# thilinarmtb/lsbench

Measured on AMD Instinct MI355X. Metric: cg_solves_per_sec, higher is better.
Workload: dtype f64

## Files before the change

lsbench_amd/csrc/hip_kernels.hip:

```cpp
#include "hip_kcommon.h"

__device__ __forceinline__ void spmv_publish(double *__restrict__ partials, double dot,
                                             double *sred, const lsb_ar_tail &tail) {
  if (!partials)
    return;
  double d[1] = {dot};
  wg_sum<1>(d, sred);
  if (tail.counter)
    ar_tail(partials, d[0], tail);
  else if (threadIdx.x == 0)
    partials[blockIdx.x] = d[0];
}

enum { SP_PREFETCH = 1, SP_NT = 2 };

template <int FLAGS, class T>
__device__ __forceinline__ T stream_load(const T *p) {
  if (FLAGS & SP_NT)
    return __builtin_nontemporal_load(p);
  return *p;
}

#define LSB_ISSUE_BLOCK(kk)                                                    \
  do {                                                                         \
    r0 = rowblk[kk], r1 = rowblk[(kk) + 1];                                    \
    j0 = offs[r0], j1 = offs[r1];                                              \
    if (j1 - j0 <= CAP) {                                                      \
      _Pragma("unroll") for (int u = 0; u < U; u++) {                          \
        const int t = (int)tid + u * WG;                                       \
        if (t < j1 - j0) {                                                     \
          c[u] = stream_load<FLAGS>(cols + j0 + t);                            \
          v[u] = stream_load<FLAGS>(vals + j0 + t);                            \
        }                                                                      \
      }                                                                        \
    }                                                                          \
  } while (0)

template <int CAP, int FLAGS, class VT = double>
__global__ __launch_bounds__(WG, 8) void k_spmv_adaptive(
    const int *__restrict__ rowblk, const unsigned char *__restrict__ blklanes,
    unsigned nblk, const int *__restrict__ offs, const int *__restrict__ cols,
    const VT *__restrict__ vals, const double *__restrict__ x,
    double *__restrict__ y, const double *__restrict__ xdot,
    double *__restrict__ partials, const lsb_pcg_state *__restrict__ st,
    const int *__restrict__ rowmap, const lsb_ar_tail tail) {
  __shared__ double sprod[CAP];
  __shared__ double sred[4];
  const unsigned tid = threadIdx.x;
  const unsigned gx = gridDim.x / NXCD;
  const unsigned xcd = blockIdx.x % NXCD, slot = blockIdx.x / NXCD;
  const unsigned chunk = (nblk + NXCD - 1) / NXCD;
  const unsigned kbeg = xcd * chunk, kend = min(kbeg + chunk, nblk);
  constexpr int U = CAP / WG;
  double dot = 0.0;
  int c[U];
  VT v[U];
  int r0 = 0, r1 = 0, j0 = 0, j1 = 0;
  unsigned k = kbeg + slot;
  if (k < kend)
    LSB_ISSUE_BLOCK(k);
  if (st && st->status)
    return;
  for (; k < kend; k += gx) {
    const int cr0 = r0, cj0 = j0, cnt = j1 - j0, nr = r1 - r0;
    if (cnt <= CAP) {
#pragma unroll
      for (int u = 0; u < U; u++) {
        const int t = (int)tid + u * WG;
        if (t < cnt)
          sprod[t] = (double)v[u] * x[c[u]];
      }
      if ((FLAGS & SP_PREFETCH) && k + gx < kend)
        LSB_ISSUE_BLOCK(k + gx);
      __syncthreads();
      unsigned L;
      if (blklanes) {
        L = blklanes[k];
      } else {
        L = 1;
        while (L < 64 && (unsigned)nr * (L * 2) <= WG)
          L <<= 1;
      }
      const unsigned sl = tid / L, l = tid % L, slots = WG / L;
      for (unsigned rb = 0; rb < (unsigned)nr; rb += slots) {
        const unsigned r = rb + sl;
        double s = 0.0;
        if (r < (unsigned)nr) {
          const int a = offs[cr0 + r] - cj0, b = offs[cr0 + r + 1] - cj0;
          for (int j = a + (int)l; j < b; j += (int)L)
            s += sprod[j];
        }
        for (unsigned off = L >> 1; off > 0; off >>= 1)
          s += __shfl_xor(s, off, 64);
        if (r < (unsigned)nr && l == 0) {
          if (rowmap) {
            y[rowmap[cr0 + r]] += s;
          } else {
            y[cr0 + r] = s;
            if (xdot)
              dot += s * xdot[cr0 + r];
          }
        }
      }
      __syncthreads();
    } else {
      double s[1] = {0.0};
      for (int j = cj0 + (int)tid; j < cj0 + cnt; j += WG)
        s[0] += (double)vals[j] * x[cols[j]];
      wg_sum<1>(s, sred);
      if (tid == 0) {
        if (rowmap) {
          y[rowmap[cr0]] += s[0];
        } else {
          y[cr0] = s[0];
          if (xdot)
            dot += s[0] * xdot[cr0];
        }
      }
      if ((FLAGS & SP_PREFETCH) && k + gx < kend)
        LSB_ISSUE_BLOCK(k + gx);
    }
    if (!(FLAGS & SP_PREFETCH) && k + gx < kend)
      LSB_ISSUE_BLOCK(k + gx);
  }
  spmv_publish(partials, dot, sred, tail);
}
#undef LSB_ISSUE_BLOCK

template <int L, class VT = double>
__global__ __launch_bounds__(WG) void k_spmv_subwave(
    unsigned n, unsigned rows_per_wg, const int *__restrict__ offs,
    const int *__restrict__ cols, const VT *__restrict__ vals,
    const double *__restrict__ x, double *__restrict__ y,
    const double *__restrict__ xdot, double *__restrict__ partials,
    const lsb_pcg_state *__restrict__ st) {
  __shared__ double sred[4];
  const unsigned tid = threadIdx.x, slot = tid / L, l = tid % L;
  constexpr unsigned SLOTS = WG / L;
  const unsigned w = xcd_contiguous_wg();
  const unsigned ra = min(w * rows_per_wg, n), rb = min(ra + rows_per_wg, n);
  const int stopped = st ? st->status : 0;
  double dot = 0.0;
  for (unsigned base = ra; base < rb; base += SLOTS) {
    const unsigned r = base + slot;
    double s = 0.0, xd = 0.0;
    if (r < rb) {
      const int j0 = offs[r], j1 = offs[r + 1];
      if (xdot)
        xd = xdot[r];
      for (int j = j0 + (int)l; j < j1; j += L)
        s += (double)vals[j] * x[cols[j]];
    }
#pragma unroll
    for (int off = L >> 1; off > 0; off >>= 1)
      s += __shfl_xor(s, off, 64);
    if (stopped)
      return;
    if (r < rb && l == 0) {
      y[r] = s;
      dot += s * xd;
    }
  }
  if (stopped)
    return;
  if (partials) {
    double d[1] = {dot};
    wg_sum<1>(d, sred);
    if (tid == 0)
      partials[w] = d[0];
  }
}

template <int L>
__global__ __launch_bounds__(WG) void k_spmv_subwave_p(
    unsigned n, unsigned rows_per_wg, const int *__restrict__ offs,
    const int *__restrict__ cols, const double *__restrict__ vals,
    const double *__restrict__ r, const double *__restrict__ dinv, double dc,
    const double *__restrict__ pold, double *__restrict__ pnew, double *__restrict__ y,
    double *__restrict__ partials, lsb_pcg_state *__restrict__ st, int parity,
    const double *__restrict__ parts2, unsigned nparts2) {
  __shared__ double sred[8];
  const unsigned tid = threadIdx.x, slot = tid / L, l = tid % L;
  constexpr unsigned SLOTS = WG / L;
  const unsigned w = xcd_contiguous_wg();
  const unsigned ra = min(w * rows_per_wg, n), rb = min(ra + rows_per_wg, n);
  const int stopped = st->status;
  const double rz_old = st->rz[parity], thresh2 = st->thresh2;
  double v[2];
  wg_sum_partials<2>(parts2, nparts2, v, sred);
  if (stopped)
    return;
  const double rz_new = v[0], rr = v[1];
  const bool conv = rr <= thresh2;
  if (blockIdx.x == 0 && threadIdx.x == 0) {
    const int it = st->iters + 1;
    st->iters = it;
    st->rr = rr;
    st->rz[parity ^ 1] = rz_new;
    if (conv)
      st->status = LSB_STATUS_CONVERGED;
    else if (it >= st->maxit)
      st->status = LSB_STATUS_MAXIT;
  }
  if (conv)
    return;
  const double beta = rz_new / rz_old;
  double dot = 0.0;
  for (unsigned base = ra; base < rb; base += SLOTS) {
    const unsigned row = base + slot;
    double s = 0.0, pi = 0.0;
    if (row < rb) {
      const int j0 = offs[row], j1 = offs[row + 1];
      pi = pnew_of(dinv ? dinv[row] : dc, r[row], beta, pold[row]);
      for (int j = j0 + (int)l; j < j1; j += L) {
        const int c = cols[j];
        s += vals[j] * pnew_of(dinv ? dinv[c] : dc, r[c], beta, pold[c]);
      }
    }
#pragma unroll
    for (int off = L >> 1; off > 0; off >>= 1)
      s += __shfl_xor(s, off, 64);
    if (row < rb && l == 0) {
      pnew[row] = pi;
      y[row] = s;
      dot += s * pi;
    }
  }
  double d[1] = {dot};
  wg_sum<1>(d, sred);
  if (tid == 0)
    partials[w] = d[0];
}

__global__ __launch_bounds__(WG) void k_spmv_scalar(
    unsigned n, unsigned rows_per_wg, const int *__restrict__ offs,
    const int *__restrict__ cols, const double *__restrict__ vals,
    const double *__restrict__ x, double *__restrict__ y,
    const double *__restrict__ xdot, double *__restrict__ partials,
    const lsb_pcg_state *__restrict__ st) {
  if (st && st->status)
    return;
  __shared__ double sred[4];
  const unsigned w = xcd_contiguous_wg();
  const unsigned ra = min(w * rows_per_wg, n), rb = min(ra + rows_per_wg, n);
  double dot = 0.0;
  for (unsigned r = ra + threadIdx.x; r < rb; r += WG) {
    double s = 0.0;
    for (int j = offs[r]; j < offs[r + 1]; j++)
      s += vals[j] * x[cols[j]];
    y[r] = s;
    if (xdot)
      dot += s * xdot[r];
  }
  if (partials) {
    double d[1] = {dot};
    wg_sum<1>(d, sred);
    if (threadIdx.x == 0)
      partials[w] = d[0];
  }
}

struct sell_deal {
  unsigned turns, base, L, period, full, total, colturns;
};
__device__ __forceinline__ sell_deal sell_deal_init(unsigned ns, unsigned period, unsigned xcd) {
  sell_deal d;
  d.period = period, d.full = 0, d.total = 0, d.colturns = 0;
  if (!period) {
    const unsigned ngrp = (ns + 3) / 4, chunk = (ngrp + NXCD - 1) / NXCD;
    const unsigned g0 = min(xcd * chunk, ngrp), g1 = min(g0 + chunk, ngrp);
    d.base = g0 * 4, d.turns = g1 - g0, d.L = 0;
  } else {
    const unsigned qlo = period * xcd / NXCD, qhi = period * (xcd + 1) / NXCD;
    const unsigned planes = ns / period, rem = ns % period;
    d.L = qhi - qlo, d.base = qlo;
    d.full = d.L * planes;
    d.total = d.full + (rem > qlo ? min(qhi, rem) - qlo : 0u);
    d.colturns = (planes / 4) * d.L;
    d.turns = d.colturns + (d.total - 4 * d.colturns + 3) / 4;
  }
  return d;
}
__device__ __forceinline__ unsigned sell_deal_slice(const sell_deal &d, unsigned it, unsigned wave,
                                                    unsigned ns) {
  if (!d.period) {
    const unsigned si = d.base + it * 4 + wave;
    return si < ns ? si : 0xFFFFFFFFu;
  }
  if (it < d.colturns)
    return ((it / d.L) * 4 + wave) * d.period + d.base + it % d.L;
  const unsigned m = it * 4 + wave;
  if (m >= d.total)
    return 0xFFFFFFFFu;
  if (m < d.full)
    return (m / d.L) * d.period + d.base + m % d.L;
  return (ns / d.period) * d.period + d.base + (m - d.full);
}

typedef int i2v __attribute__((ext_vector_type(2)));
typedef int i4v __attribute__((ext_vector_type(4)));
typedef double sell_d2u __attribute__((ext_vector_type(2), aligned(8)));
typedef double sell_d2v __attribute__((ext_vector_type(2)));
#define SELL_U 5
template <class VT> struct vt2;
template <> struct vt2<double> { typedef double type __attribute__((ext_vector_type(2))); };
template <> struct vt2<float> { typedef float type __attribute__((ext_vector_type(2))); };
template <int FLAGS, class VT = double>
__global__ __launch_bounds__(WG, 6) void k_spmv_sell(
    const unsigned *__restrict__ sptr, unsigned s0, unsigned ns, unsigned period, unsigned n,
    const int *__restrict__ cols, const VT *__restrict__ vals,
    const double *__restrict__ x, double *__restrict__ y, const double *__restrict__ xdot,
    double *__restrict__ partials, const lsb_pcg_state *__restrict__ st, const lsb_ar_tail tail) {
  __shared__ double sred[4];
  const unsigned tid = threadIdx.x, lane = tid & 63u, wave = tid >> 6;
  const unsigned gx = gridDim.x / NXCD, xcd = blockIdx.x % NXCD, slot = blockIdx.x / NXCD;
  const sell_deal deal = sell_deal_init(ns, period, xcd);
  const int stopped = st ? st->status : 0;
  double dot = 0.0;
  for (unsigned g = slot; g < deal.turns; g += gx) {
    const unsigned si = __builtin_amdgcn_readfirstlane(sell_deal_slice(deal, g, wave, ns));
    if (si != 0xFFFFFFFFu) {
      const unsigned s = s0 + si;
      const unsigned base = sptr[s], len = (sptr[s + 1] - base) / LSB_SELL_ROWS;
      typedef typename vt2<VT>::type v2t;
      const i2v *cp = (const i2v *)(cols + base) + lane;
      const v2t *vp = (const v2t *)(vals + base) + lane;
      double a0 = 0.0, a1 = 0.0;
      for (unsigned j0 = 0; j0 < len; j0 += SELL_U) {
        i2v c[SELL_U];
        v2t v[SELL_U];
#pragma unroll
        for (int u = 0; u < SELL_U; u++)
          if (j0 + u < len) {
            if (FLAGS & SP_NT) {
              c[u] = __builtin_nontemporal_load(cp + (size_t)(j0 + u) * 64);
              v[u] = __builtin_nontemporal_load(vp + (size_t)(j0 + u) * 64);
            } else {
              c[u] = cp[(size_t)(j0 + u) * 64];
              v[u] = vp[(size_t)(j0 + u) * 64];
            }
          }
        if (stopped)
          return;
#pragma unroll
        for (int u = 0; u < SELL_U; u++)
          if (j0 + u < len) {
            a0 = fma((double)v[u].x, x[c[u].x], a0);
            a1 = fma((double)v[u].y, x[c[u].y], a1);
          }
      }
      const unsigned row = s * LSB_SELL_ROWS + 2 * lane;
      if (row + 1 < n) {
        const sell_d2v o = {a0, a1};
        *(sell_d2v *)(y + row) = o;
        if (xdot) {
          dot = fma(a0, xdot[row], dot);
          dot = fma(a1, xdot[row + 1], dot);
        }
      } else if (row < n) {
        y[row] = a0;
        if (xdot)
          dot = fma(a0, xdot[row], dot);
      }
    }
  }
  if (stopped)
    return;
  spmv_publish(partials, dot, sred, tail);
}

typedef short s2v __attribute__((ext_vector_type(2)));
template <int FLAGS, class VT = double, bool CHEB = false>
__global__ __launch_bounds__(WG, 6) void k_spmv_sell16(
    const unsigned *__restrict__ sptr, unsigned s0, unsigned ns, unsigned period, unsigned n,
    unsigned row_begin, unsigned xlen, const short *__restrict__ codes, const int *__restrict__ sbase,
    const VT *__restrict__ vals, const double *__restrict__ vconst, unsigned ulen,
    const double *__restrict__ x, double *__restrict__ y, const double *__restrict__ xdot,
    double *__restrict__ partials,
    const lsb_pcg_state *__restrict__ st, const lsb_ar_tail tail, const lsb_cheb_epi epi) {
  __shared__ double sred[4];
  const unsigned tid = threadIdx.x, lane = tid & 63u, wave = tid >> 6;
  const unsigned gx = gridDim.x / NXCD, xcd = blockIdx.x % NXCD, slot = blockIdx.x / NXCD;
  const sell_deal deal = sell_deal_init(ns, period, xcd);
  const int stopped = st ? st->status : 0;
  double dot = 0.0;
  for (unsigned g = slot; g < deal.turns; g += gx) {
    const unsigned si = __builtin_amdgcn_readfirstlane(sell_deal_slice(deal, g, wave, ns));
    if (si != 0xFFFFFFFFu) {
      const unsigned s = s0 + si;
      typedef typename vt2<VT>::type v2t;
      const unsigned base = ulen ? s * ulen * LSB_SELL_ROWS : sptr[s];
      const unsigned len = ulen ? ulen : (sptr[s + 1] - base) / LSB_SELL_ROWS;
      const unsigned q0 = base / LSB_SELL_ROWS;
      const unsigned row = s * LSB_SELL_ROWS + 2 * lane;
      const int grow = (int)(row + row_begin);
      double a0 = 0.0, a1 = 0.0;
      sell_d2v xd = {0.0, 0.0};
      if (!CHEB && xdot) {
        if (row + 1 < n)
          xd = *(const sell_d2v *)(xdot + row);
        else if (row < n)
          xd.x = xdot[row];
      }
      for (unsigned j0 = 0; j0 < len; j0 += SELL_U) {
        if (vconst) {
          const unsigned cnt = len - j0 < SELL_U ? len - j0 : SELL_U;
          i4v rec[SELL_U];
          double cst[SELL_U];
#pragma unroll
          for (int u = 0; u < SELL_U; u++) {
            const unsigned q = q0 + j0 + ((unsigned)u < cnt ? (unsigned)u : cnt - 1u);
            rec[u] = ((const i4v *)sbase)[q];
            cst[u] = vconst[q];
          }
          bool fast = true;
#pragma unroll
          for (int u = 0; u < SELL_U; u++)
            fast = fast && (rec[u].y < 0 && rec[u].z < 0);
          if (fast) {
            if (stopped)
              return;
            sell_d2u t[SELL_U];
#pragma unroll
            for (int u = 0; u < SELL_U; u++)
              t[u] = *(const sell_d2u *)(x + (grow + rec[u].x));
#pragma unroll
            for (int u = 0; u < SELL_U; u++)
              if ((unsigned)u < cnt) {
                const VT cv = (VT)cst[u];
// ... 1332 lines not shown
```

Measured before the change: 1.159.

## Prefetch row offsets and lane counts for next block in adaptive SpMV

Splits the block-issue macro into metadata and stream parts, and computes the lane log2 for the next block ahead of time (reading blklanes via readfirstlane). It also prefetches each thread's row offsets for the first two reduction passes into registers, which takes the dependent offs loads off the critical path after the barrier. x gathers are batched in groups of four so more loads are in flight at once. In exchange it uses more registers, which may lower occupancy, and the group loop assumes U is a multiple of GB.

```diff
diff --git a/lsbench_amd/csrc/hip_kernels.hip b/lsbench_amd/csrc/hip_kernels.hip
--- a/lsbench_amd/csrc/hip_kernels.hip
+++ b/lsbench_amd/csrc/hip_kernels.hip
@@ -21,10 +21,20 @@
   return *p;
 }
 
-#define LSB_ISSUE_BLOCK(kk)                                                    \
+#define LSB_ISSUE_META(kk)                                                     \
   do {                                                                         \
     r0 = rowblk[kk], r1 = rowblk[(kk) + 1];                                    \
     j0 = offs[r0], j1 = offs[r1];                                              \
+    if (blklanes) {                                                            \
+      lg = (unsigned)__ffs(__builtin_amdgcn_readfirstlane((int)blklanes[kk])) - 1u;  \
+    } else {                                                                   \
+      lg = 0;                                                                  \
+      while (lg < 6 && ((unsigned)(r1 - r0) << (lg + 1)) <= WG)                \
+        lg++;                                                                  \
+    }                                                                          \
+  } while (0)
+#define LSB_ISSUE_STREAM()                                                     \
+  do {                                                                         \
     if (j1 - j0 <= CAP) {                                                      \
       _Pragma("unroll") for (int u = 0; u < U; u++) {                          \
         const int t = (int)tid + u * WG;                                       \
@@ -33,6 +43,23 @@
           v[u] = stream_load<FLAGS>(vals + j0 + t);                            \
         }                                                                      \
       }                                                                        \
+    }                                                                          \
+  } while (0)
+
+#define LSB_ISSUE_BLOCK(kk)                                                    \
+  do {                                                                         \
+    LSB_ISSUE_META(kk);                                                        \
+    LSB_ISSUE_STREAM();                                                        \
+  } while (0)
+
+#define LSB_ISSUE_OFFS()                                                       \
+  do {                                                                         \
+    if (j1 - j0 <= CAP) {                                                      \
+      const unsigned rows = (unsigned)(r1 - r0), sn = tid >> lg, step = WG >> lg; \
+      if (sn < rows)                                                           \
+        ro[0] = offs[r0 + sn], ro[1] = offs[r0 + sn + 1];                      \
+      if (sn + step < rows)                                                    \
+        ro[2] = offs[r0 + sn + step], ro[3] = offs[r0 + sn + step + 1];        \
     }                                                                          \
   } while (0)
 
@@ -52,41 +79,51 @@
   const unsigned chunk = (nblk + NXCD - 1) / NXCD;
   const unsigned kbeg = xcd * chunk, kend = min(kbeg + chunk, nblk);
   constexpr int U = CAP / WG;
+  constexpr int GB = 4;
   double dot = 0.0;
-  int c[U];
+  int c[U] = {};
   VT v[U];
+  int ro[4] = {0, 0, 0, 0};
   int r0 = 0, r1 = 0, j0 = 0, j1 = 0;
+  unsigned lg = 0;
   unsigned k = kbeg + slot;
-  if (k < kend)
+  if (k < kend) {
     LSB_ISSUE_BLOCK(k);
+    LSB_ISSUE_OFFS();
+  }
   if (st && st->status)
     return;
   for (; k < kend; k += gx) {
     const int cr0 = r0, cj0 = j0, cnt = j1 - j0, nr = r1 - r0;
+    const unsigned clg = lg;
     if (cnt <= CAP) {
 #pragma unroll
-      for (int u = 0; u < U; u++) {
-        const int t = (int)tid + u * WG;
-        if (t < cnt)
-          sprod[t] = (double)v[u] * x[c[u]];
+      for (int h = 0; cnt > 0 && h < U; h += GB) {
+        double xv[GB];
+#pragma unroll
+        for (int u = 0; u < GB; u++)
+          xv[u] = x[c[h + u]];
+#pragma unroll
+        for (int u = 0; u < GB; u++) {
+          const int t = (int)tid + (h + u) * WG;
+          if (t < cnt)
+            sprod[t] = (double)v[h + u] * xv[u];
+        }
       }
       if ((FLAGS & SP_PREFETCH) && k + gx < kend)
         LSB_ISSUE_BLOCK(k + gx);
       __syncthreads();
-      unsigned L;
-      if (blklanes) {
-        L = blklanes[k];
-      } else {
-        L = 1;
-        while (L < 64 && (unsigned)nr * (L * 2) <= WG)
-          L <<= 1;
-      }
-      const unsigned sl = tid / L, l = tid % L, slots = WG / L;
-      for (unsigned rb = 0; rb < (unsigned)nr; rb += slots) {
+      const unsigned L = 1u << clg, sl = tid >> clg, l = tid & (L - 1u), slots = WG >> clg;
+      unsigned pass = 0;
+      for (unsigned rb = 0; rb < (unsigned)nr; rb += slots, pass++) {
         const unsigned r = rb + sl;
         double s = 0.0;
         if (r < (unsigned)nr) {
-          const int a = offs[cr0 + r] - cj0, b = offs[cr0 + r + 1] - cj0;
+          int a, b;
+          if (pass < 2)
+            a = (pass ? ro[2] : ro[0]) - cj0, b = (pass ? ro[3] : ro[1]) - cj0;
+          else
+            a = offs[cr0 + r] - cj0, b = offs[cr0 + r + 1] - cj0;
           for (int j = a + (int)l; j < b; j += (int)L)
             s += sprod[j];
         }
@@ -121,10 +158,17 @@
         LSB_ISSUE_BLOCK(k + gx);
     }
     if (!(FLAGS & SP_PREFETCH) && k + gx < kend)
-      LSB_ISSUE_BLOCK(k + gx);
+      LSB_ISSUE_META(k + gx);
+    if (k + gx < kend)
+      LSB_ISSUE_OFFS();
+    if (!(FLAGS & SP_PREFETCH) && k + gx < kend)
+      LSB_ISSUE_STREAM();
   }
   spmv_publish(partials, dot, sred, tail);
 }
+#undef LSB_ISSUE_OFFS
+#undef LSB_ISSUE_META
+#undef LSB_ISSUE_STREAM
 #undef LSB_ISSUE_BLOCK
 
 template <int L, class VT = double>
```

Measured after the change: 1.158. Within noise of the previous version (-0.1%).
